# natir/br

Hardware: AMD Instinct MI355X
Metric: corrected Gbases/sec at k=19, 10 kb ONT-error reads (higher is better)
Workload: dtype u64 k-mers / 1-bit set

## Files before the change

br_amd/csrc/brx_correct.hip:

```cpp
#include "brx_correct.hpp"
#include <chrono>

#include <stdlib.h>
#include <string.h>
#include <algorithm>
#include <type_traits>
#include <thread>
#include <vector>

using namespace brx;

namespace brx {
uint64_t scan_tmp_bytes(uint32_t n);
int exclusive_scan_lens(const uint32_t *d_lens, uint32_t n, uint64_t *d_tmp, uint64_t *d_out_offsets,
                        unsigned long long *d_total, hipStream_t s);
int upload_batch(const uint8_t *bases, const uint64_t *offsets, uint32_t n_reads, uint8_t **d_bases, uint64_t *bases_cap,
                 uint64_t **d_off, uint64_t *off_cap, uint64_t *total, hipStream_t stream);
}

namespace {

enum { ST_INIT = 0, ST_SCAN, ST_ERRLEN, ST_ALTS, ST_SCEN, ST_MORE, ST_WALK, ST_T1, ST_TSCORE, ST_TMORE, ST_GFOLLOW, ST_GVALID };
enum { MODE_ONE = 0, MODE_GRAPH = 1, MODE_INSSUB = 2, MODE_TWO = 3 };

// ... 340 lines not shown
            }
            const uint64_t s0 = slot_of(o0, r, p.slack), s1 = slot_of(o1, (uint64_t)r + 1, p.slack);
            out = p.out + s0;
            cap = (uint32_t)(s1 - s0);
            st = ST_INIT;
            i = 0;
            olen = 0;
            kmer = 0;
            prev = false;
            steps = 0;
            skip_until = 0;
            if (VERIFY) {
                i = tr.i;
                olen = tr.i;
                uint64_t km = 0;
                for (int j = 0; j < k; j++)
                    km = (km << 2) | nuc2bit(in[p.flip ? (n - 1u - (tr.i + 1u - (uint32_t)k + (uint32_t)j)) : (tr.i + 1u - (uint32_t)k + (uint32_t)j)]);
                kmer = km;
                ch_t = in[p.flip ? (n - 1u - tr.i) : tr.i];
                elen = tr.elen;
                fc = tr.fc;
                if (HAS_TWO)
                    mode = MODE_TWO;
                else if (M == BRX_GRAPH)
                    mode = MODE_GRAPH;
                else if (M == BRX_GAP_SIZE) {
                    mode = elen < (uint32_t)k ? MODE_GRAPH : (elen == (uint32_t)k ? MODE_ONE : MODE_INSSUB);
                    gap = elen > (uint32_t)k ? elen - (uint32_t)k : 0u;
                } else
                    mode = MODE_ONE;
                st = ST_ALTS;
            }
            return;
        }
    };
    auto ld = [&](uint32_t j) -> uint8_t { return in[p.flip ? (n - 1u - j) : j]; };
    int done = 0;
    bool flag_read = false;
    auto end_read = [&](int how) {
        if (VERIFY && how != 1) {
            flag_read = true;
            done = 1;
        } else {
            done = how;
        }
    };
    auto finish = [&]() { end_read(1); };
    auto overflow = [&]() { end_read(16 + CTL_OVERFLOW); };
    auto nonterminating = [&]() { end_read(16 + CTL_NONTERM); };
    auto path_overflow = [&]() { end_read(16 + CTL_PATHOVF); };
    auto lane_kmer = [&](uint64_t carry, uint64_t code) -> uint64_t {
        uint64_t val = code;
#pragma unroll
        for (int d = 1; d < G && d < 32; d <<= 1) {
            const uint64_t other = __shfl_up(val, d, G);
            if (gl >= d)
                val |= other << (2 * d);
        }
        const int nb = gl + 1;
        return (nb >= k) ? (val & mask) : (((carry << (2 * nb)) | val) & mask);
    };

    constexpr int WB = G < 32 ? G : 32;
    auto group_window = [&](uint64_t code) -> uint64_t {
        uint64_t val = code;
#pragma unroll
        for (int d = 1; d < WB; d <<= 1) {
            const uint64_t other = __shfl_up(val, d, G);
            if (gl >= d)
                val |= other << (2 * d);
        }
        return __shfl(val, gshift + WB - 1);
    };
    auto ext = [&](uint64_t km, uint64_t W, uint32_t b0, uint32_t nb) -> uint64_t {
        const uint64_t bits = (W >> (2u * ((uint32_t)WB - b0 - nb))) & ((1ull << (2u * nb)) - 1ull);
        return ((km << (2u * nb)) | bits) & mask;
    };
    uint64_t win = 0;

    fetch();

    while (__any(have)) {
        if (G == 64) {
            while (have && st == ST_SCAN && !slow && n - i >= 65u && olen + 66u <= cap) {
                const uint8_t c8 = ld(i + (uint32_t)lane);
                const uint64_t km = lane_kmer64_dpp(kmer, (uint32_t)nuc2bit(c8), lane, mask);
                bool s1 = false;
                if (HAS_ERRLEN && i + (uint32_t)lane < skip_until) {
                } else if (p.idx.lines) {
                    s1 = index_get(p.idx, p.bits, km, k);
                } else {
                    s1 = probe(p.bits, km, k);
                }
                const uint64_t bs = __ballot(s1);
                const uint64_t trig = ~bs & ((bs << 1) | (prev ? 1ull : 0ull));
                if (trig)
                    break;
                out[olen + (uint32_t)lane] = c8;
                olen += 64u;
                i += 64u;
                kmer = ((uint64_t)(uint32_t)__builtin_amdgcn_readlane((int)(uint32_t)(km >> 32), 63) << 32) |
                       (uint32_t)__builtin_amdgcn_readlane((int)(uint32_t)km, 63);
                prev = (bs >> 63) & 1ull;
                n_rounds += 1u;
                n_probes += 64u;
                steps++;
            }
            while (HAS_ERRLEN && have && st == ST_ERRLEN && !slow && n - i > ej + 1u + 64u) {
                const uint8_t c8 = ld(i + ej + 1u + (uint32_t)lane);
                const uint64_t km = lane_kmer64_dpp(ek, (uint32_t)nuc2bit(c8), lane, mask);
                const bool s1 = p.idx.lines ? index_get(p.idx, p.bits, km, k) : probe(p.bits, km, k);
                if (__ballot(s1))
                    break;
                ek = ((uint64_t)(uint32_t)__builtin_amdgcn_readlane((int)(uint32_t)(km >> 32), 63) << 32) |
                     (uint32_t)__builtin_amdgcn_readlane((int)(uint32_t)km, 63);
                ej += 64u;
                n_rounds += 1u;
                n_probes += 64u;
                steps++;
            }
        }
        if (HAS_WALK) {
            constexpr uint64_t LEADERS = G == 64 ? 1ull : (G == 32 ? 0x0000000100000001ull : (G == 16 ? 0x0001000100010001ull : (G == 8 ? 0x0101010101010101ull : 0x1111111111111111ull)));
            for (uint32_t it = 0;; it++) {
                const bool wfast = have && st == ST_WALK && !slow && (brent || mode == MODE_INSSUB);
                const uint32_t nw = (uint32_t)__builtin_popcountll(__ballot(wfast) & LEADERS);
                const uint32_t no = (uint32_t)__builtin_popcountll(__ballot(have && !wfast) & LEADERS);
                if (nw == 0u || nw < no || (no != 0u && it >= 8u))
                    break;
                bool s1 = false, u1 = false;
                if (wfast && gl < 4) {
                    const uint64_t q = add_nuc(wk, (uint64_t)gl, mask);
                    if (p.idx.lines) {
                        const int pr = index_probe(p.idx, q, k);
                        s1 = pr == 1;
                        u1 = pr == 2;
                    } else {
                        s1 = probe(p.bits, q, k);
                    }
                }
                if (__ballot(u1))
                    break;
                const uint32_t am = (uint32_t)((__ballot(s1) >> gshift) & 0xfull);
                bool simple = wfast && __popc(am) == 1;
                uint64_t nk = 0;
                if (simple) {
                    nk = add_nuc(wk, (uint64_t)(__ffs(am) - 1), mask);
                    simple = !(brent && nk == tort) && !(!brent && npath >= p.maxpath) &&
                             !(mode == MODE_GRAPH ? nk == fc : gap <= 1u) && steps < (1u << 24) + 64u * n;
                }
                if (simple) {
                    if (brent && ++blam == bpow) {
                        tort = nk;
                        bpow *= 2u;
                        blam = 0;
                    }
                    if (gl == 0 && npath < p.maxpath)
                        __hip_atomic_store(path + npath, (unsigned long long)nk, __ATOMIC_RELAXED, __HIP_MEMORY_SCOPE_AGENT);
                    if (npath < 0xfffffff0u)
                        npath++;
                    wk = nk;
                    if (mode != MODE_GRAPH)
                        gap--;
                    steps++;
                }
                n_rounds += nw;
// ... 773 lines not shown
            if (cc)
                atomicAdd(p.ctrl + CTL_TRIGGERS, (unsigned long long)cc);
            if (d)
                atomicAdd(p.ctrl + CTL_FIXES, (unsigned long long)d);
        }
        ev = 0;
        since_flush = 0;
    };

    auto fetch = [&]() {
        for (;;) {
            unsigned long long w = 0;
            if (gl == 0)
                w = atomicAdd(p.ctrl + CTL_WORK, 1ull);
            w = __shfl(w, gshift);
            if (w >= (LIST ? *p.only_n : (unsigned long long)p.n_reads)) {
                have = false;
                return;
            }
            have = true;
            r = LIST ? p.only[w] : (uint32_t)w;
            const uint64_t o0 = p.offsets[r], o1 = p.offsets[r + 1];
            if (p.in_staged) {
                in = p.in + slot_of(o0, r, p.slack);
                n = p.in_lens[r];
                if (n == 0xffffffffu) {
                    if (gl == 0)
                        p.out_lens[r] = 0xffffffffu;
                    continue;
                }
            } else {
                in = p.in + o0;
                n = (uint32_t)(o1 - o0);
            }
            const uint64_t s0 = slot_of(o0, r, p.slack), s1 = slot_of(o1, (uint64_t)r + 1, p.slack);
            out = p.out + s0;
            cap = (uint32_t)(s1 - s0);
            st = ST_INIT;
            i = 0;
            olen = 0;
            kmer = 0;
            prev = false;
            steps = 0;
            return;
        }
    };
    auto ld = [&](uint32_t j) -> uint8_t { return in[p.flip ? (n - 1u - j) : j]; };
    int done = 0;
    auto finish = [&]() { done = 1; };
    auto give_up = [&](int which) { done = 16 + which; };
    auto lane_kmer = [&](uint64_t carry, uint32_t code, uint32_t &scan_out) -> uint64_t {
        if (G == 4) {
            const uint32_t v = row_scan4(code) & ((1u << nb2) - 1u);
            scan_out = v;
            return ((carry << nb2) | v) & mask;
        } else if (G == 8) {
            const uint32_t v = row_scan8(code) & ((1u << nb2) - 1u);
            scan_out = v;
            return ((carry << nb2) | v) & mask;
        } else if (G == 16) {
            const uint32_t v = row_scan16(code);
            scan_out = v;
            return ((carry << nb2) | v) & mask;
        } else {
            scan_out = 0;
            return lane_kmer64_dpp(carry, code, lane, mask);
        }
    };
    auto ext = [&](uint64_t km, uint32_t b0, uint32_t nb) -> uint64_t {
        const uint64_t bits = (uint64_t)((win >> (2u * ((uint32_t)WB - b0 - nb))) & (decltype(win))((1ull << (2u * nb)) - 1ull));
        return ((km << (2u * nb)) | bits) & mask;
    };

    fetch();

    while (__any(have)) {
        lane = lane0;
        asm volatile("" : "+v"(lane));
        gl = lane & (G - 1);
        gshift = lane & ~(G - 1);
        bcast_addr = (uint32_t)(lane | (G - 1)) * 4u;
        nb2 = 2u * ((uint32_t)gl + 1u);
        if (G == 64) {
            while (have && st == ST_SCAN && !slow && n - i >= 65u && olen + 66u <= cap) {
                const uint8_t c8 = ld(i + (uint32_t)lane);
                uint32_t sc;
                const uint64_t km = lane_kmer(kmer, (uint32_t)nuc2bit(c8), sc);
                const bool s1 = p.idx.lines ? index_get(p.idx, p.bits, km, k) : probe(p.bits, km, k);
                const uint64_t bs = __ballot(s1);
                const uint64_t trig = ~bs & ((bs << 1) | (prev ? 1ull : 0ull));
                if (trig)
                    break;
                out[olen + (uint32_t)lane] = c8;
                olen += 64u;
                i += 64u;
                kmer = ((uint64_t)(uint32_t)__builtin_amdgcn_readlane((int)(uint32_t)(km >> 32), 63) << 32) |
                       (uint32_t)__builtin_amdgcn_readlane((int)(uint32_t)km, 63);
                prev = (bs >> 63) & 1ull;
                ev += ((lane == 0) ? 1u : 0u) + (1u << 8);
                steps++;
                if (++since_flush == 255u)
                    flush();
            }
        }
        bool do_probe = false;
        uint64_t pk = 0;
        uint8_t ch = 0;
        uint32_t sc_s = 0, scan = 0, gwin = 0;
        bool sc_active = false;

        if (have) {
            ev += (gl == 0) ? 1u : 0u;
            if (st == ST_SCAN) {
                const uint32_t pos = i + (uint32_t)gl;
                const bool valid = pos < n;
                if (G < 64)
                    ch = pf_ch;
                else
                    ch = valid ? ld(pos) : (uint8_t)0;
                pk = lane_kmer(kmer, (uint32_t)nuc2bit(ch), scan);
                do_probe = valid;
                if (G <= 16)
                    gwin = (uint32_t)__builtin_amdgcn_ds_bpermute((int)bcast_addr, (int)scan);
            } else if (st == ST_INIT) {
                if (n < (uint32_t)k) {
                    for (uint32_t j = gl; j < n; j += G)
                        out[j] = ld(j);
                    olen = n;
                } else {
                    uint64_t km = 0;
                    for (int j = 0; j < k; j++)
                        km = (km << 2) | nuc2bit(ld((uint32_t)j));
                    kmer = km;
                    for (uint32_t j = gl; j < (uint32_t)k; j += G)
                        out[j] = ld(j);
                    olen = (uint32_t)k;
                    i = (uint32_t)k;
                    do_probe = (gl == 0);
                    pk = kmer;
                }
            } else if (st == ST_ALTS) {
                do_probe = gl < 4 && (uint64_t)gl != (kmer & 3ull);
                pk = (kmer & ~3ull) | (uint64_t)gl;
                if (G == 4) {
                    const uint32_t w4 = i + 4u * (uint32_t)gl;
                    uint32_t raw = 0;
                    if (w4 + 4u <= n) {
                        const uint8_t *q = p.flip ? in + (n - 4u - w4) : in + w4;
                        __builtin_memcpy(&raw, q, 4);
                        if (p.flip)
                            raw = __builtin_bswap32(raw);
                    } else {
                        for (uint32_t t = 0; t < 4u && w4 + t < n; t++)
                            raw |= (uint32_t)ld(w4 + t) << (8u * t);
                    }
                    uint32_t v = ((((raw >> 1) & 0x03030303u) * 0x40100401u) >> 24);
                    v |= dpp_row_shr<1>(v) << 8;
                    v |= dpp_row_shr<2>(v) << 16;
                    if (gl != 3)
                        v &= (1u << (8u * ((uint32_t)gl + 1u))) - 1u;
                    win = (uint32_t)__builtin_amdgcn_ds_bpermute((int)bcast_addr, (int)v);
                }
                const uint32_t wp = i + (uint32_t)gl;
                const uint32_t cd = (G != 4 && gl < WB && wp < n) ? (uint32_t)nuc2bit(ld(wp)) : 0u;
                if (G == 4) {
                } else if (G == 8) {
                    const uint32_t v = row_scan8(cd) & ((1u << nb2) - 1u);
                    win = (uint32_t)__builtin_amdgcn_ds_bpermute((int)bcast_addr, (int)v);
                } else if (G == 16) {
                    win = (uint32_t)__builtin_amdgcn_ds_bpermute((int)bcast_addr, (int)row_scan16(cd));
                } else {
                    const uint32_t v = row_scan16(cd);
                    const uint32_t w0 = (uint32_t)__builtin_amdgcn_readlane((int)v, 15), w1 = (uint32_t)__builtin_amdgcn_readlane((int)v, 31);
                    win = ((uint64_t)w0 << 32) | w1;
                }
            } else if (st == ST_SCEN && (G == 8 || G == 16)) {
                uint32_t off, j;
                if (sub == 0u) {
                    sc_s = (uint32_t)gl >> 1;
                    j = (uint32_t)gl & 1u;
                    sc_active = gl < 6 && !((failmask >> sc_s) & 1u) && j < c;
                } else {
                    sc_s = (uint32_t)__ffs(7u & ~failmask & ~passmask) - 1u;
                    j = sub + (uint32_t)gl;
                    sc_active = j < c;
                }
                off = 2u - sc_s;
                if (sc_active) {
                    if (c + 3u <= (uint32_t)WB) {
                        pk = ext(corr, off, j + 1u);
                    } else {
                        pk = corr;
                        for (uint32_t q = 0; q <= j; q++)
                            pk = add_nuc(pk, nuc2bit(ld(i + off + q)), mask);
                    }
                    do_probe = true;
                }
            } else if (st == ST_SCEN) {
                const uint32_t width = scen_width(sub, c, G, 0u, failmask);
                const uint32_t e = (uint32_t)gl;
                const uint32_t alive = ~failmask & 7u;
                const uint32_t ord = (e >= width ? 1u : 0u) + (e >= 2u * width ? 1u : 0u);
                sc_active = e < 3u * width && ord < (uint32_t)__popc(alive);
                const uint32_t a1 = alive & (alive - 1u);
                sc_s = !sc_active ? 0u : (ord == 0u ? (uint32_t)__ffs(alive) - 1u : (ord == 1u ? (uint32_t)__ffs(a1) - 1u : 2u));
                const uint32_t j = sub + (sc_active ? e - ord * width : 0u);
                const uint32_t off = 2u - sc_s;
                if (sc_active) {
                    if (c + 3u <= (uint32_t)WB) {
                        pk = ext(corr, off, j + 1u);
                    } else {
                        pk = corr;
                        for (uint32_t q = 0; q <= j; q++)
                            pk = add_nuc(pk, nuc2bit(ld(i + off + q)), mask);
                    }
                    do_probe = true;
                }
            } else {
// ... 202 lines not shown
                if (__popc(keep) == 1)
                    apply_s = __ffs(keep) - 1;
                else
                    fail = true;
            }
            if (have && steps > (1u << 24) + 64u * n) {
                fail = false;
                apply_s = -1;
                give_up(CTL_NONTERM);
            }
            if (fail) {
                if (olen + 2u > cap) {
                    give_up(CTL_OVERFLOW);
                } else {
                    if (gl == 0)
                        out[olen] = ld(i);
                    olen += 1;
                    i += 1;
                    prev = false;
                    if (i >= n)
                        finish();
                    else
                        st = ST_SCAN;
                }
            } else if (apply_s >= 0) {
                if (olen + 2u > cap) {
                    give_up(CTL_OVERFLOW);
                } else {
                    if (gl == 0)
                        out[olen] = bit2nuc(corr & 3ull);
                    olen += 1;
                    kmer = corr;
                    prev = true;
                    const uint32_t off = 2u - (uint32_t)apply_s;
                    i += off;
                    ev += (gl == 0) ? (1u << 24) : 0u;
                    if (c > 0u && c + 3u <= (uint32_t)WB && olen + c + 1u <= cap) {
                        for (uint32_t q = (uint32_t)gl; q < c; q += (uint32_t)G)
                            out[olen + q] = ld(i + q);
                        kmer = ext(kmer, off, c);
                        olen += c;
                        i += c;
                    }
                    if (i >= n)
                        finish();
                    else
                        st = ST_SCAN;
                }
            }
        }
        if (G < 64 && have && !done && !retry && st == ST_SCAN) {
            const uint32_t pos = i + (uint32_t)gl;
            pf_ch = pos < n ? ld(pos) : (uint8_t)0;
        }
        if (done) {
            if (gl == 0) {
                p.out_lens[r] = done == 1 ? olen : 0xffffffffu;
                if (done != 1)
                    atomicAdd(p.ctrl + (done - 16), 1ull);
            }
            done = 0;
            fetch();
        }
        if (++since_flush == 255u)
            flush();
    }
    flush();
}

#ifndef BRX_REV_WAVES
#define BRX_REV_WAVES 7
#endif
template <int KT, int M>
__global__ __launch_bounds__(256, BRX_REV_WAVES) void rev_scan_kernel(const PassParams pp, uint32_t *__restrict__ handback, uint32_t *__restrict__ redo_flag,
                                                                          TrigRec *__restrict__ notes, uint32_t trig_cap)
{
    const IdxView idx = pp.idx;
    const uint32_t *const bits = pp.bits;
    unsigned long long *const ctrl = pp.ctrl;
    const uint32_t n_reads = pp.n_reads, slack = pp.slack;
    const uint64_t *const offsets = pp.offsets;
    const uint8_t *const in_base = pp.in;
    const uint32_t *const in_lens = pp.in_lens;
    const bool in_staged = pp.in_staged != 0, flip = pp.flip != 0;
    uint8_t *const out_base = pp.out;
    uint32_t *const out_lens = pp.out_lens;
    constexpr bool HAS_ERRLEN = (M == BRX_GRAPH || M == BRX_GAP_SIZE);
    const int lane = threadIdx.x & 63;
    const int k = KT ? KT : pp.k;
    const uint64_t mask = kmask(k);
    uint32_t n_rounds = 0, n_probes = 0, n_trig = 0;

    auto ask = [&](uint64_t km) __attribute__((always_inline)) -> bool { return idx.lines ? index_get(idx, bits, km, k) : probe(bits, km, k); };
    auto last_of = [&](uint64_t km, uint32_t l) __attribute__((always_inline)) -> uint64_t {
        return ((uint64_t)(uint32_t)__builtin_amdgcn_readlane((int)(uint32_t)(km >> 32), (int)l) << 32) |
               (uint32_t)__builtin_amdgcn_readlane((int)(uint32_t)km, (int)l);
    };

    for (;;) {
        unsigned long long w = 0;
        if (lane == 0)
            w = atomicAdd(ctrl + CTL_WORK, 1ull);
        const uint32_t r = (uint32_t)__builtin_amdgcn_readfirstlane((int)(uint32_t)w);
        if (__builtin_amdgcn_readfirstlane((int)(uint32_t)(w >> 32)) != 0 || r >= n_reads)
            break;
        const uint64_t o0 = offsets[r], o1 = offsets[r + 1];
        const uint8_t *in;
        uint32_t n;
        if (in_staged) {
            in = in_base + slot_of(o0, r, slack);
            n = in_lens[r];
            if (n == 0xffffffffu) {
                if (lane == 0)
                    out_lens[r] = 0xffffffffu;
                continue;
            }
        } else {
            in = in_base + o0;
            n = (uint32_t)(o1 - o0);
        }
        const uint64_t s0 = slot_of(o0, r, slack), s1 = slot_of(o1, (uint64_t)r + 1, slack);
        uint8_t *out = out_base + s0;
        const uint32_t cap = (uint32_t)(s1 - s0);
        auto ld = [&](uint32_t j) __attribute__((always_inline)) -> uint8_t { return in[flip ? (n - 1u - j) : j]; };

        if (n < (uint32_t)k) {
            for (uint32_t j = (uint32_t)lane; j < n; j += 64u)
                out[j] = ld(j);
            if (lane == 0)
                out_lens[r] = n;
            continue;
        }
        bool hb = n + 1u > cap;
        uint64_t kmer = 0;
        uint32_t i = (uint32_t)k, skip_until = 0, trig_read = 0;
        bool prev = false;
        if (!hb) {
            for (int j = 0; j < k; j++)
                kmer = (kmer << 2) | nuc2bit(ld((uint32_t)j));
            if (lane < k)
                out[lane] = ld((uint32_t)lane);
            prev = ask(kmer);
            n_rounds++;
            n_probes++;
        }
        while (!hb && i < n) {
            const uint32_t pos = i + (uint32_t)lane;
            const bool valid = pos < n;
            const uint8_t c8 = valid ? ld(pos) : (uint8_t)0;
            const uint64_t km = lane_kmer64_dpp(kmer, (uint32_t)nuc2bit(c8), lane, mask);
            const bool asks = valid && !(HAS_ERRLEN && pos < skip_until);
            const bool a1 = asks && ask(km);
            n_rounds++;
            n_probes += (uint32_t)__builtin_popcountll(__ballot(asks));
            const uint32_t left = n - i;
            const uint32_t cnt = left < 64u ? left : 64u;
            const uint64_t vmask = cnt >= 64u ? ~0ull : ((1ull << cnt) - 1ull);
            const uint64_t bs = __ballot(a1);
            const uint64_t trig = ~bs & ((bs << 1) | (prev ? 1ull : 0ull)) & vmask;
            if (!trig) {
                if (valid)
                    out[pos] = c8;
                kmer = last_of(km, cnt - 1u);
                prev = (bs >> (cnt - 1u)) & 1ull;
                i += cnt;
                continue;
            }
            const uint32_t t = (uint32_t)__builtin_ctzll(trig);
            if ((uint32_t)lane < t)
                out[pos] = c8;
            i += t;
            kmer = last_of(km, t);
            trig_read++;
            uint32_t elen = 0;
            uint64_t fc = 0;
            bool hit_end = false;
            if (HAS_ERRLEN) {
                uint64_t ek = kmer;
                uint32_t ej = 0;
                const uint32_t rem = n - i;
                for (;;) {
                    const uint32_t j = ej + 1u + (uint32_t)lane;
                    const bool v2 = j < rem;
                    const uint8_t c2 = v2 ? ld(i + j) : (uint8_t)0;
                    const uint64_t km2 = lane_kmer64_dpp(ek, (uint32_t)nuc2bit(c2), lane, mask);
                    const bool a2 = v2 && ask(km2);
                    n_rounds++;
                    n_probes += (uint32_t)__builtin_popcountll(__ballot(v2));
                    const uint64_t sm = __ballot(a2);
                    if (sm) {
                        const uint32_t t2 = (uint32_t)__builtin_ctzll(sm);
                        elen = ej + 1u + t2;
                        fc = last_of(km2, t2);
                        break;
                    }
                    if (rem <= ej + 1u + 64u) {
                        const uint32_t nv = rem - (ej + 1u);
                        elen = rem;
                        fc = nv ? last_of(km2, nv - 1u) : ek;
                        hit_end = true;
                        break;
                    }
                    ek = last_of(km2, 63u);
                    ej += 64u;
                }
            }
            const bool none_already = HAS_ERRLEN && hit_end && (M == BRX_GRAPH || elen < (uint32_t)k);
            if (!none_already) {
                const bool asks3 = lane < 4 && (uint64_t)lane != (kmer & 3ull);
                const bool a3 = asks3 && ask(add_nuc(kmer >> 2, (uint64_t)(lane & 3), mask));
                n_rounds++;
                n_probes += 3u;
                if (__builtin_popcountll(__ballot(a3)) == 1) {
                    unsigned long long at = 0;
                    if (lane == 0)
                        at = atomicAdd(ctrl + CTL_REV_TRIGS, 1ull);
                    const uint32_t at_lo = (uint32_t)__builtin_amdgcn_readfirstlane((int)(uint32_t)at);
                    if (__builtin_amdgcn_readfirstlane((int)(uint32_t)(at >> 32)) != 0 || at_lo >= trig_cap) {
                        hb = true;
                        break;
                    }
                    if (lane == 0) {
                        notes[at_lo] = TrigRec{r, i, elen, 0u, fc};
                        atomicAdd(ctrl + CTL_REV_TRIGS_SUM, 1ull);
                    }
                }
            }
            if (lane == 0)
                out[i] = ld(i);
// ... 220 lines not shown
                correct_kernel<8, M, 2><<<blocks, 256, lds, s>>>(p);
            return BRX_OK;
        }
        if (p.only) {
            correct_kernel<64, M, 1><<<blocks, 256, lds, s>>>(p);
            return BRX_OK;
        }
    }
    if (lds > 64 * 1024) {
        const void *fn = G == 16 ? (const void *)correct_kernel<16, M>
                       : G == 32 ? (const void *)correct_kernel<32, M> : (const void *)correct_kernel<64, M>;
        BRX_HIP(hipFuncSetAttribute(fn, hipFuncAttributeMaxDynamicSharedMemorySize, (int)lds));
    }
    if (G <= 8 && M == BRX_ONE)
        correct_kernel<8, BRX_ONE><<<blocks, 256, lds, s>>>(p);
    else if (G == 4 && (M == BRX_GRAPH || M == BRX_GAP_SIZE))
        correct_kernel<4, (M == BRX_GRAPH || M == BRX_GAP_SIZE) ? M : BRX_GRAPH><<<blocks, 256, lds, s>>>(p);
    else if (G == 8 && (M == BRX_GRAPH || M == BRX_GAP_SIZE))
        correct_kernel<8, (M == BRX_GRAPH || M == BRX_GAP_SIZE) ? M : BRX_GRAPH><<<blocks, 256, lds, s>>>(p);
    else if (G <= 16)
        correct_kernel<16, M><<<blocks, 256, lds, s>>>(p);
    else if (G == 32)
        correct_kernel<32, M><<<blocks, 256, lds, s>>>(p);
    else
        correct_kernel<64, M><<<blocks, 256, lds, s>>>(p);
    return BRX_OK;
}

int greedy_group(int G, int k, int max_search, uint32_t *dim, uint32_t *per_group)
{
    *dim = (uint32_t)(k + max_search + 2);
    *per_group = greedy_lds_bytes(*dim);
    for (; G <= 64; G *= 2)
        if ((uint64_t)(256 / G) * *per_group <= 160u * 1024u)
            return G;
    return 0;
}

int launch_pass(PassParams p, const brx_method_t &md, int G, hipStream_t s)
{
    static const char *names[5] = {"correct_pass", "correct_pass_two", "correct_pass_graph", "correct_pass_greedy",
                                   "correct_pass_gap_size"};
    const int method = md.method;
    size_t lds = 0;
    p.max_search = md.max_search;
    {
        const char *e = getenv("BRX_TUNE");
        p.flags = e ? (uint32_t)atoi(e) : 0u;
    }
    p.g_dim = 0;
    p.g_lds_bytes = 0;
    if (method == BRX_GREEDY) {
        G = greedy_group(G, p.k, md.max_search, &p.g_dim, &p.g_lds_bytes);
        if (!G) {
            set_error("greedy: k=%d with max_search=%d needs a %u x %u alignment table that does not fit LDS", p.k,
                      (int)md.max_search, p.g_dim, p.g_dim);
            return BRX_ERR_UNSUPPORTED;
        }
        lds = (size_t)(256 / G) * p.g_lds_bytes;
    }
    uint32_t blocks = pass_blocks(p.n_reads, G, method == BRX_ONE);
    if (p.only || p.trig) {
        const uint64_t sized_groups = sized_path_lists(p.n_reads);
        const uint32_t per_block = p.trig ? 256u / (uint32_t)verify_group() : 4u;
        blocks = (uint32_t)(sized_groups / per_block);
        blocks = blocks < 1u ? 1u : (blocks > MAX_BLOCKS ? MAX_BLOCKS : blocks);
    }
    KernelTimer t(p.trig ? "rev_verify" : (p.only ? "rev_redo" : names[method]), s);
    switch (method) {
    case BRX_ONE: BRX_TRY(launch_method<BRX_ONE>(p, G, blocks, lds, s)); break;
    case BRX_TWO: BRX_TRY(launch_method<BRX_TWO>(p, G, blocks, lds, s)); break;
    case BRX_GRAPH: BRX_TRY(launch_method<BRX_GRAPH>(p, G, blocks, lds, s)); break;
    case BRX_GREEDY: BRX_TRY(launch_method<BRX_GREEDY>(p, G, blocks, lds, s)); break;
    case BRX_GAP_SIZE: BRX_TRY(launch_method<BRX_GAP_SIZE>(p, G, blocks, lds, s)); break;
    default: break;
    }
    BRX_HIP(hipGetLastError());
    return BRX_OK;
}

bool rev_lean_on()
{
    const char *e = getenv("BRX_REV_LEAN");
    return !(e && *e == '0');
}

template <int M>
void launch_rev_scan(const PassParams &p, uint32_t *list, uint32_t *flag, TrigRec *trig, uint32_t trig_cap, uint32_t blocks, hipStream_t s)
{
    if (p.k == 19)
        rev_scan_kernel<19, M><<<blocks, 256, 0, s>>>(p, list, flag, trig, trig_cap);
    else if (p.k == 21)
        rev_scan_kernel<21, M><<<blocks, 256, 0, s>>>(p, list, flag, trig, trig_cap);
    else
        rev_scan_kernel<0, M><<<blocks, 256, 0, s>>>(p, list, flag, trig, trig_cap);
}

int launch_rev_lean(brx_chain *ch, PassParams p, const brx_method_t &md, hipStream_t s)
{
    static const char *names[5] = {"correct_pass", "correct_pass_two", "correct_pass_graph", "correct_pass_greedy",
                                   "correct_pass_gap_size"};
    const uint64_t trig_cap64 = 4ull * p.n_reads + 4096ull;
    const uint32_t trig_cap = trig_cap64 > 0x7fffffffull ? 0x7fffffffu : (uint32_t)trig_cap64;
    BRX_TRY(ensure((void **)&ch->d_rev_list, &ch->rev_list_bytes, (uint64_t)p.n_reads * 4ull));
    BRX_TRY(ensure((void **)&ch->d_rev_flag, &ch->rev_flag_bytes, (uint64_t)p.n_reads * 4ull));
    BRX_TRY(ensure(&ch->d_rev_trig, &ch->rev_trig_bytes, (uint64_t)trig_cap * sizeof(TrigRec)));
    BRX_HIP(hipMemsetAsync(p.ctrl + CTL_REV_HANDBACK, 0, 8, s));
    BRX_HIP(hipMemsetAsync(p.ctrl + CTL_REV_TRIGS, 0, 8, s));
    BRX_HIP(hipMemsetAsync(ch->d_rev_flag, 0, (uint64_t)p.n_reads * 4ull, s));
    TrigRec *trig = (TrigRec *)ch->d_rev_trig;
    {
        const uint32_t blocks = pass_blocks(p.n_reads, 64);
        KernelTimer t(names[md.method], s);
        switch (md.method) {
        case BRX_ONE: launch_rev_scan<BRX_ONE>(p, ch->d_rev_list, ch->d_rev_flag, trig, trig_cap, blocks, s); break;
        case BRX_GRAPH: launch_rev_scan<BRX_GRAPH>(p, ch->d_rev_list, ch->d_rev_flag, trig, trig_cap, blocks, s); break;
        case BRX_GAP_SIZE: launch_rev_scan<BRX_GAP_SIZE>(p, ch->d_rev_list, ch->d_rev_flag, trig, trig_cap, blocks, s); break;
        default: set_error("launch_rev_lean: method %u", md.method); return BRX_ERR_ARG;
        }
        BRX_HIP(hipGetLastError());
    }
    PassParams v = p;
    v.trig = trig;
    v.trig_cap = trig_cap;
    v.only_n = p.ctrl + CTL_REV_TRIGS;
    v.redo_list = ch->d_rev_list;
    v.redo_flag = ch->d_rev_flag;
    BRX_HIP(hipMemsetAsync(p.ctrl + CTL_WORK, 0, 8, s));
    BRX_TRY(launch_pass(v, md, 16, s));
    p.only = ch->d_rev_list;
    p.only_n = p.ctrl + CTL_REV_HANDBACK;
    BRX_HIP(hipMemsetAsync(p.ctrl + CTL_WORK, 0, 8, s));
    return launch_pass(p, md, 16, s);
}

}

extern "C" {

int brx_chain_new(const brx_set_t *set, const brx_method_t *methods, uint32_t n_methods, bool two_side,
                  brx_chain_t **out)
{
    return brx_chain_new_pass(set, methods, n_methods, two_side ? BRX_PASS_NONE : BRX_PASS_REVERSE, out);
}

int brx_chain_second_pass(const brx_chain_t *ch)
{
    if (!ch) {
        set_error("null argument");
        return BRX_ERR_ARG;
    }
    return ch->second_pass;
}

int brx_chain_new_pass(const brx_set_t *set, const brx_method_t *methods, uint32_t n_methods, int second_pass,
                       brx_chain_t **out)
{
    if (!set || !out || (!methods && n_methods)) {
        set_error("null argument");
        return BRX_ERR_ARG;
    }
    if (second_pass != BRX_PASS_NONE && second_pass != BRX_PASS_REVERSE && second_pass != BRX_PASS_REVCOMP) {
        set_error("unknown second-pass mode %d (0 none, 1 reverse, 2 revcomp)", second_pass);
        return BRX_ERR_ARG;
    }
    for (uint32_t m = 0; m < n_methods; m++)
// ... 182 lines not shown
                BRX_TRY(ensure_bits(ch->set, s, "correction"));
                break;
            }
    BRX_TRY(index_ensure(ch->set, s));
    IdxView idx{nullptr, 0, 0, 0};
    if (ch->set->idx_valid && (index_wanted(k) || no_bits(ch->set)))
        idx = IdxView{ch->set->d_lines, 32u - ch->set->idx_log_lines, ch->set->idx_m, (uint32_t)k - ch->set->idx_m + 1u,
                      ch->set->idx_linebits ? (const uint32_t *)(ch->set->d_lines + (8ull << ch->set->idx_log_lines)) : nullptr};
    if (const char *e = getenv("BRX_LINE_BITS"))
        if (*e == '0')
            idx.line_bits = nullptr;

    const int n_dirs = ch->two_side ? 1 : 2;
    const bool revcomp = ch->second_pass == BRX_PASS_REVCOMP;
    const int n_methods = (int)ch->methods.size();
    uint64_t stats[8] = {0, 0, 0, 0, 0, 0, 0, 0};
    std::vector<SideRead> side;
    const int G = group_width(false, idx.lines != nullptr, n_reads);
    bool needs_path = false;
    for (int m = 0; m < n_methods; m++)
        needs_path |= (ch->methods[m].method == BRX_GRAPH || ch->methods[m].method == BRX_GAP_SIZE ||
                       ch->methods[m].method == BRX_GREEDY);
    uint32_t maxpath = ch->maxpath_seen;

    for (uint32_t slack = ch->slack_seen, attempt = 0;; attempt++) {
        if (attempt > 12) {
            set_error("correction output / graph walks do not fit the workspace after 12 enlargements; giving up");
            return BRX_ERR_OVERFLOW;
        }
        if (needs_path) {
            const uint64_t n_groups = sized_path_lists(n_reads);
            BRX_TRY(ensure((void **)&ch->d_path, &ch->path_bytes, n_groups * maxpath * 8ull));
        }
        const uint64_t stage_need = total_bases + (total_bases >> 2) * slack + 64ull * ((uint64_t)n_reads + 1) + 64;
        if (stage_need > ch->stage_bytes || !ch->d_stage[0]) {
            for (int q = 0; q < 2; q++) {
                if (ch->d_stage[q])
                    (void)hipFree(ch->d_stage[q]);
                ch->d_stage[q] = nullptr;
            }
            ch->stage_bytes = 0;
            BRX_HIP(hipMalloc((void **)&ch->d_stage[0], stage_need));
            BRX_HIP(hipMalloc((void **)&ch->d_stage[1], stage_need));
            ch->stage_bytes = stage_need;
        }

        const uint8_t *cur = d_bases;
        const uint32_t *cur_lens = nullptr;
        int cur_staged = 0, cur_rev = 0, pp = 0;
        bool any_overflow = false;
        BRX_HIP(hipMemsetAsync(ch->d_ctrl, 0, CTL_N * 8, s));
        for (int scan = 0; scan < n_dirs && !any_overflow; scan++) {
            const int dir = revcomp ? 0 : scan;
            if (revcomp && scan == 1 && cur_staged) {
                revcomp_stage(cur, cur_lens, d_offsets, n_reads, slack, ch->d_stage[pp], ch->d_lens[pp], s);
                cur = ch->d_stage[pp];
                cur_lens = ch->d_lens[pp];
                pp ^= 1;
            }
            for (int m = 0; m < n_methods; m++) {
                PassParams p;
                p.bits = no_bits(ch->set) ? nullptr : ch->set->d_bits;
                const int mth = ch->methods[m].method;
                const char *e_fwd = getenv("BRX_INDEX_FWD");
                const unsigned idx_fwd = e_fwd ? (unsigned)atoi(e_fwd) : 29u;
                const bool use_idx = no_bits(ch->set) || ((idx_fwd >> mth) & 1u) || (dir == 1 && mth != BRX_GREEDY);
                p.idx = use_idx ? idx : IdxView{nullptr, 0, 0, 0};
                p.k = k;
                p.c = ch->methods[m].confirm;
                p.n_reads = n_reads;
                p.offsets = d_offsets;
                p.in = cur;
                p.in_lens = cur_lens;
                p.in_staged = cur_staged;
                p.flip = (cur_rev != dir);
                p.out = ch->d_stage[pp];
                p.out_lens = ch->d_lens[pp];
                p.slack = slack;
                p.ctrl = (unsigned long long *)ch->d_ctrl;
                p.path_k = ch->d_path;
                p.maxpath = maxpath;
                BRX_HIP(hipMemsetAsync(ch->d_ctrl + CTL_WORK, 0, 8, s));
                p.flags = 0;
                p.max_search = 0;
                p.g_dim = 0;
                p.g_lds_bytes = 0;
                const unsigned lane_rev_default = 0u;
                const char *e_rev = getenv("BRX_LANE_REV");
                const unsigned lane_rev = e_rev && *e_rev ? (unsigned)atoi(e_rev) : lane_rev_default;
                const bool lane_dir = dir == 0 ? !p.flip
                                               : ((mth == BRX_GRAPH && (lane_rev & 1u)) || (mth == BRX_GAP_SIZE && (lane_rev & 2u)));
                if ((mth == BRX_ONE || mth == BRX_GRAPH || mth == BRX_GAP_SIZE) && lane_dir) {
                    const LanePassInfo info{cur_staged ? ch->stage_bytes : total_bases, mth};
                    const int lst = lane_pass(ch, p, info, s);
                    if (lst != BRX_OK && lst != BRX_ERR_UNSUPPORTED)
                        return lst;
                    if (lst == BRX_OK) {
                        cur = ch->d_stage[pp];
                        cur_lens = ch->d_lens[pp];
                        cur_staged = 1;
                        cur_rev = dir;
                        pp ^= 1;
                        continue;
                    }
                }
                int gw = dir ? group_width(true, false, n_reads) : G;
                if (gw < 16 && mth != BRX_ONE) {
                    gw = (mth == BRX_GRAPH || mth == BRX_GAP_SIZE) ? walk_group() : 16;
                }
                const char *e_lo = getenv("BRX_REV_LEAN_ONE");
                const bool lean_one = mth == BRX_ONE && e_lo && *e_lo == '1';
                const bool lean = dir == 1 && (mth == BRX_GRAPH || mth == BRX_GAP_SIZE || lean_one) && gw == 64 && rev_lean_on();
                if (lean)
                    BRX_TRY(launch_rev_lean(ch, p, ch->methods[m], s));
                else
                    BRX_TRY(launch_pass(p, ch->methods[m], gw, s));
                cur = ch->d_stage[pp];
                cur_lens = ch->d_lens[pp];
                cur_staged = 1;
                cur_rev = dir;
                pp ^= 1;
            }
        }
        if (n_methods == 0) {
            set_error("empty method list");
            return BRX_ERR_ARG;
        }
        static const bool tr_attempts = [] { const char *e = getenv("BRX_TRACE"); return e && *e == '1'; }();
        if (tr_attempts)
            fprintf(stderr, "[brx correct] attempt %u launched: slack %u maxpath %u n_reads %u\n", attempt, slack, maxpath, n_reads);
        BRX_HIP(hipMemcpyAsync(ch->h_ctrl, ch->d_ctrl, CTL_N * 8, hipMemcpyDeviceToHost, s));
        BRX_HIP(hipStreamSynchronize(s));
        if (tr_attempts)
            fprintf(stderr, "[brx correct] attempt %u done: slot overflows %llu, walk list overflows %llu, nonterminating %llu, "
                            "lean reverse passes: %llu open triggers verified, %llu reads redone\n", attempt,
                    (unsigned long long)ch->h_ctrl[CTL_OVERFLOW], (unsigned long long)ch->h_ctrl[CTL_PATHOVF],
                    (unsigned long long)ch->h_ctrl[CTL_NONTERM], (unsigned long long)ch->h_ctrl[CTL_REV_TRIGS_SUM],
                    (unsigned long long)ch->h_ctrl[CTL_REV_HANDBACK_SUM]);
        stats[4] = attempt;
        if (ch->h_ctrl[CTL_NONTERM] != 0) {
            set_error("%llu read(s): the scan does not terminate (e.g. greedy moving the read cursor backwards for ever; "
                      "the reference spins on such input)", (unsigned long long)ch->h_ctrl[CTL_NONTERM]);
            return BRX_ERR_UNSUPPORTED;
        }
        if (ch->h_ctrl[CTL_OVERFLOW] != 0 || ch->h_ctrl[CTL_PATHOVF] != 0) {
            stats[5] += ch->h_ctrl[CTL_OVERFLOW];
            stats[6] += ch->h_ctrl[CTL_PATHOVF];
            bool patched = false;
            if (ch->h_ctrl[CTL_OVERFLOW] + ch->h_ctrl[CTL_PATHOVF] <= redo_max_reads()) {
                side.clear();
                const int rst = redo_poisoned_reads(ch, d_bases, d_offsets, n_reads, const_cast<uint8_t *>(cur),
                                                    const_cast<uint32_t *>(cur_lens), cur_rev, slack,
                                                    ch->h_ctrl[CTL_OVERFLOW] ? slack * 4u : slack,
                                                    ch->h_ctrl[CTL_PATHOVF] ? maxpath * 8u : maxpath, side, s);
                if (rst == BRX_OK) {
                    patched = true;
                    if (ch->sub)
                        for (int q = 0; q < 4; q++)
                            stats[q] += ch->sub->last_stats[q];
                }
                else if (rst != BRX_ERR_UNSUPPORTED)
                    return rst;
            }
            if (!patched) {
                side.clear();
                if (ch->h_ctrl[CTL_OVERFLOW] != 0)
// ... 277 lines not shown
```

br_amd/csrc/brx_correct.hpp:

```cpp
#pragma once
#include "brx_internal.hpp"
#include "brx_index.hpp"

namespace brx {

enum { CTL_WORK = 0, CTL_OVERFLOW = 1, CTL_ROUNDS = 2, CTL_PROBES = 3, CTL_TRIGGERS = 4, CTL_FIXES = 5, CTL_TOTAL = 6, CTL_PATHOVF = 7, CTL_NONTERM = 8,
       CTL_LANE_UNITS = 9, CTL_LANE_MISS = 10, CTL_LANE_WORK = 11, CTL_LANE_FAIL = 12,
       CTL_REV_HANDBACK = 13, CTL_REV_HANDBACK_SUM = 14,
       CTL_LANE_UNWRITTEN = 15,
       CTL_REV_TRIGS = 16, CTL_REV_TRIGS_SUM = 17,
       CTL_AP_VEC = 18, CTL_AP_BYTEWAY = 19, CTL_AP_PARTIAL = 20,
       CTL_N = 21 };

struct TrigRec {
    uint32_t r;
    uint32_t i;
    uint32_t elen;
    uint32_t pad;
    uint64_t fc;
};

struct PassParams {
    const uint32_t *bits;
    IdxView idx;
    int k;
    int c;
    uint32_t n_reads;
    const uint64_t *offsets;
    const uint8_t *in;
    const uint32_t *in_lens;
    int in_staged;
    int flip;
    uint8_t *out;
    uint32_t *out_lens;
    uint32_t slack;
    unsigned long long *ctrl;
    uint64_t *path_k;
    uint32_t maxpath;
    uint32_t flags;
    int max_search;
    uint32_t g_dim;
    uint32_t g_lds_bytes;
    const uint32_t *only = nullptr;
    const unsigned long long *only_n = nullptr;
    const TrigRec *trig = nullptr;
    uint32_t trig_cap = 0;
    uint32_t *redo_list = nullptr;
    uint32_t *redo_flag = nullptr;
};

__host__ __device__ __forceinline__ uint64_t slot_of(uint64_t o, uint64_t r, uint32_t slack)
{
    return o + (o >> 2) * (uint64_t)slack + 64ull * r;
}

__device__ __forceinline__ bool probe(const uint32_t *__restrict__ bits, uint64_t fwd, int k)
{
    const uint64_t h = khash(fwd, k);
    return (bits[h >> 5] >> (h & 31u)) & 1u;
}


#if defined(__HIPCC__)
template <int D>
__device__ __forceinline__ uint32_t dpp_row_shr(uint32_t v)
{
    return (uint32_t)__builtin_amdgcn_update_dpp(0, (int)v, 0x110 + D, 0xf, 0xf, true);
}

__device__ __forceinline__ uint32_t row_scan16(uint32_t code)
{
    uint32_t v = code;
    v |= dpp_row_shr<1>(v) << 2;
    v |= dpp_row_shr<2>(v) << 4;
    v |= dpp_row_shr<4>(v) << 8;
    v |= dpp_row_shr<8>(v) << 16;
    return v;
}
__device__ __forceinline__ uint64_t lane_kmer64_dpp(uint64_t carry, uint32_t code, int lane, uint64_t mask)
{
    const uint32_t v = row_scan16(code);
    const uint32_t clo = (uint32_t)carry, chi = (uint32_t)(carry >> 32);
    const uint32_t b1 = (uint32_t)__builtin_amdgcn_update_dpp((int)clo, (int)v, 0x142 , 0xe, 0xf, false);
    const uint32_t old2 = (lane < 16) ? chi : clo;
    const uint32_t b2 = (uint32_t)__builtin_amdgcn_update_dpp((int)old2, (int)b1, 0x142, 0xc, 0xf, false);
    const uint32_t jb = 2u * ((uint32_t)(lane & 15) + 1u);
    return (((((uint64_t)b2 << 32) | b1) << jb) | v) & mask;
}

#endif

struct LanePassInfo {
    uint64_t in_total_bound;
    int method;
};
int lane_pass(brx_chain *ch, const PassParams &p, const LanePassInfo &info, hipStream_t s);
void lane_ws_free(brx_chain *ch);
int launch_one_list(const PassParams &p, hipStream_t s);
int launch_walk_list(const PassParams &p, int method, hipStream_t s);

}
```

Before: 26.65.

## Batch reverse-pass scan rounds with minimizer prefilter and compacted probe queue

Adds a block path for the reverse-direction scan. It processes several 64-base rounds per call, computes minimizer line hashes with DPP, and filters k-mers through a line-occupancy bitmap. Only surviving k-mers are compacted into an LDS queue and probed in dense waves, which cuts divergent index probes per round. The cost is possible wasted work when a trigger appears early in the block, plus extra LDS use. The change also builds the initial k-mer with a wave-parallel DPP scan in place of a serial loop.

```diff
diff --git a/br_amd/csrc/brx_correct.hip b/br_amd/csrc/brx_correct.hip
--- a/br_amd/csrc/brx_correct.hip
+++ b/br_amd/csrc/brx_correct.hip
@@ -446,6 +446,22 @@
 
     while (__any(have)) {
         if (G == 64) {
+            while (!HAS_GREEDY && p.rev_batch && have && st == ST_SCAN && !slow && n - i >= 64u * REV_BLOCK + 1u && olen + 64u * REV_BLOCK + 2u <= cap) {
+                const uint8_t *const in_b = (const uint8_t *)uni64((uint64_t)in);
+                uint8_t *const out_b = (uint8_t *)uni64((uint64_t)(out + olen));
+                const uint32_t n_b = uni32(n), i_b = uni32(i);
+                const bool flip_b = p.flip != 0;
+                const uint32_t t = rev_block_rounds<HAS_ERRLEN>(p.idx, p.bits, k, mask, lane,
+                                                                [in_b, n_b, flip_b](uint32_t j) -> uint8_t { return in_b[flip_b ? (n_b - 1u - j) : j]; }, i_b,
+                                                                out_b, uni32(skip_until), kmer, prev);
+                olen += 64u * t;
+                i += 64u * t;
+                n_rounds += t;
+                n_probes += 64u * t;
+                steps += t;
+                if (t < (uint32_t)REV_BLOCK)
+                    break;
+            }
             while (have && st == ST_SCAN && !slow && n - i >= 65u && olen + 66u <= cap) {
                 const uint8_t c8 = ld(i + (uint32_t)lane);
                 const uint64_t km = lane_kmer64_dpp(kmer, (uint32_t)nuc2bit(c8), lane, mask);
@@ -1385,6 +1401,24 @@
         bcast_addr = (uint32_t)(lane | (G - 1)) * 4u;
         nb2 = 2u * ((uint32_t)gl + 1u);
         if (G == 64) {
+            while (p.rev_batch && have && st == ST_SCAN && !slow && n - i >= 64u * REV_BLOCK + 1u && olen + 64u * REV_BLOCK + 2u <= cap) {
+                if (since_flush + REV_BLOCK >= 255u)
+                    flush();
+                const uint8_t *const in_b = (const uint8_t *)uni64((uint64_t)in);
+                uint8_t *const out_b = (uint8_t *)uni64((uint64_t)(out + olen));
+                const uint32_t n_b = uni32(n), i_b = uni32(i);
+                const bool flip_b = p.flip != 0;
+                const uint32_t t = rev_block_rounds<false>(p.idx, p.bits, k, mask, lane,
+                                                           [in_b, n_b, flip_b](uint32_t j) -> uint8_t { return in_b[flip_b ? (n_b - 1u - j) : j]; }, i_b,
+                                                           out_b, 0u, kmer, prev);
+                olen += 64u * t;
+                i += 64u * t;
+                ev += ((lane == 0) ? t : 0u) + (t << 8);
+                steps += t;
+                since_flush += t;
+                if (t < (uint32_t)REV_BLOCK)
+                    break;
+            }
             while (have && st == ST_SCAN && !slow && n - i >= 65u && olen + 66u <= cap) {
                 const uint8_t c8 = ld(i + (uint32_t)lane);
                 uint32_t sc;
@@ -1431,12 +1465,21 @@
                         out[j] = ld(j);
                     olen = n;
                 } else {
-                    uint64_t km = 0;
-                    for (int j = 0; j < k; j++)
-                        km = (km << 2) | nuc2bit(ld((uint32_t)j));
-                    kmer = km;
-                    for (uint32_t j = gl; j < (uint32_t)k; j += G)
-                        out[j] = ld(j);
+                    if (G == 64) {
+                        const uint8_t cj = lane < k ? ld((uint32_t)lane) : (uint8_t)0;
+                        const uint64_t kv = lane_kmer64_dpp(0ull, (uint32_t)nuc2bit(cj), lane, mask);
+                        kmer = ((uint64_t)(uint32_t)__builtin_amdgcn_readlane((int)(uint32_t)(kv >> 32), k - 1) << 32) |
+                               (uint32_t)__builtin_amdgcn_readlane((int)(uint32_t)kv, k - 1);
+                        if (lane < k)
+                            out[lane] = cj;
+                    } else {
+                        uint64_t km = 0;
+                        for (int j = 0; j < k; j++)
+                            km = (km << 2) | nuc2bit(ld((uint32_t)j));
+                        kmer = km;
+                        for (uint32_t j = gl; j < (uint32_t)k; j += G)
+                            out[j] = ld(j);
+                    }
                     olen = (uint32_t)k;
                     i = (uint32_t)k;
                     do_probe = (gl == 0);
@@ -1805,7 +1848,7 @@
     const uint64_t *const offsets = pp.offsets;
     const uint8_t *const in_base = pp.in;
     const uint32_t *const in_lens = pp.in_lens;
-    const bool in_staged = pp.in_staged != 0, flip = pp.flip != 0;
+    const bool in_staged = pp.in_staged != 0, flip = pp.flip != 0, rev_batch = pp.rev_batch != 0;
     uint8_t *const out_base = pp.out;
     uint32_t *const out_lens = pp.out_lens;
     constexpr bool HAS_ERRLEN = (M == BRX_GRAPH || M == BRX_GAP_SIZE);
@@ -1868,6 +1911,20 @@
             n_probes++;
         }
         while (!hb && i < n) {
+            if (rev_batch && n - i >= 64u * REV_BLOCK + 1u) {
+                const uint32_t t = rev_block_rounds<HAS_ERRLEN>(idx, bits, k, mask, lane,
+                                                                [in, n, flip](uint32_t j) -> uint8_t { return in[flip ? (n - 1u - j) : j]; }, i,
+                                                                out + i, skip_until, kmer, prev);
+                for (uint32_t q = 0; q < t; q++) {
+                    const uint32_t p0 = i + 64u * q;
+                    const uint32_t skipped = (HAS_ERRLEN && skip_until > p0) ? (skip_until - p0 < 64u ? skip_until - p0 : 64u) : 0u;
+                    n_probes += 64u - skipped;
+                }
+                n_rounds += t;
+                i += 64u * t;
+                if (t == (uint32_t)REV_BLOCK)
+                    continue;
+            }
             const uint32_t pos = i + (uint32_t)lane;
             const bool valid = pos < n;
             const uint8_t c8 = valid ? ld(pos) : (uint8_t)0;
@@ -2254,6 +2311,12 @@
 bool rev_lean_on()
 {
     const char *e = getenv("BRX_REV_LEAN");
+    return !(e && *e == '0');
+}
+
+bool rev_batch_on()
+{
+    const char *e = getenv("BRX_REV_BATCH");
     return !(e && *e == '0');
 }
 
@@ -2602,6 +2665,7 @@
                 p.maxpath = maxpath;
                 BRX_HIP(hipMemsetAsync(ch->d_ctrl + CTL_WORK, 0, 8, s));
                 p.flags = 0;
+                p.rev_batch = (dir == 1 && !revcomp && rev_batch_on() && rev_block_applies(p.idx)) ? 1 : 0;
                 p.max_search = 0;
                 p.g_dim = 0;
                 p.g_lds_bytes = 0;
diff --git a/br_amd/csrc/brx_correct.hpp b/br_amd/csrc/brx_correct.hpp
--- a/br_amd/csrc/brx_correct.hpp
+++ b/br_amd/csrc/brx_correct.hpp
@@ -47,6 +47,7 @@
     uint32_t trig_cap = 0;
     uint32_t *redo_list = nullptr;
     uint32_t *redo_flag = nullptr;
+    int rev_batch = 0;
 };
 
 __host__ __device__ __forceinline__ uint64_t slot_of(uint64_t o, uint64_t r, uint32_t slack)
@@ -87,7 +88,143 @@
     const uint32_t jb = 2u * ((uint32_t)(lane & 15) + 1u);
     return (((((uint64_t)b2 << 32) | b1) << jb) | v) & mask;
 }
-
+#endif
+
+#ifndef BRX_REV_BLOCK
+#define BRX_REV_BLOCK 4
+#endif
+constexpr int REV_BLOCK = BRX_REV_BLOCK;
+constexpr uint32_t REV_MAX_W = 8;
+constexpr uint32_t REV_QUEUE = 128;
+static_assert(REV_BLOCK >= 1 && REV_BLOCK <= 16, "BRX_REV_BLOCK: 1 .. 16 rounds");
+
+inline bool rev_block_applies(const IdxView &v)
+{
+    return v.lines != nullptr && v.line_bits != nullptr && v.line_shift >= 6u && v.w >= 1u && v.w <= REV_MAX_W;
+}
+
+#if defined(__HIPCC__)
+__device__ __forceinline__ uint32_t mmer_hash(uint32_t f, uint32_t m)
+{
+    uint32_t x = __brev(f ^ 0xAAAAAAAAu);
+    x = ((x >> 1) & 0x55555555u) | ((x & 0x55555555u) << 1);
+    const uint32_t r = x >> (32u - 2u * m);
+    return (f < r ? f : r) * 0x9E3779B1u;
+}
+
+__device__ __forceinline__ uint32_t uni32(uint32_t v) { return (uint32_t)__builtin_amdgcn_readfirstlane((int)v); }
+__device__ __forceinline__ uint64_t uni64(uint64_t v) { return ((uint64_t)uni32((uint32_t)(v >> 32)) << 32) | uni32((uint32_t)v); }
+
+template <bool HAS_SKIP, typename LD>
+__device__ __forceinline__ uint32_t rev_block_rounds(const IdxView &idx, const uint32_t *__restrict__ bits, int k, uint64_t mask, int lane0, LD ld,
+                                                     uint32_t i, uint8_t *__restrict__ outp, uint32_t skip_until, uint64_t &kmer, bool &prev)
+{
+    __shared__ uint4 rev_q[4][REV_QUEUE];
+    __shared__ unsigned long long rev_ans[4][2 * REV_BLOCK];
+    const uint32_t wv = uni32(threadIdx.x >> 6);
+    uint4 *const q = rev_q[wv];
+    unsigned long long *const ans = rev_ans[wv];
+    unsigned long long *const carry = ans + REV_BLOCK;
+    const uint32_t m = idx.m, w = idx.w;
+    const uint32_t mm = m >= 16u ? 0xffffffffu : (1u << (2u * m)) - 1u;
+
+    if (lane0 < REV_BLOCK)
+        ans[lane0] = 0ull;
+
+    uint32_t count = 0;
+    bool any_solid = false;
+    uint64_t cur_carry = uni64(kmer);
+    uint8_t c_next = ld(i + (uint32_t)lane0);
+#pragma unroll 1
+    for (uint32_t r = 0; r < (uint32_t)REV_BLOCK; r++) {
+        {
+            int ln = lane0;
+            asm volatile("" : "+v"(ln));
+            const uint8_t c8 = c_next;
+            if (r + 1u < (uint32_t)REV_BLOCK)
+                c_next = ld(i + 64u * (r + 1u) + (uint32_t)ln);
+            const uint64_t carry_in = cur_carry;
+            const uint64_t km = lane_kmer64_dpp(cur_carry, (uint32_t)nuc2bit(c8), ln, mask);
+            outp[64u * r + (uint32_t)ln] = c8;
+            if (ln == 63)
+                carry[r] = km;
+            cur_carry = ((uint64_t)(uint32_t)__builtin_amdgcn_readlane((int)(uint32_t)(km >> 32), 63) << 32) |
+                        (uint32_t)__builtin_amdgcn_readlane((int)(uint32_t)km, 63);
+            const uint32_t h = mmer_hash((uint32_t)km & mm, m);
+            uint32_t best = h, cur = h;
+#pragma unroll
+            for (uint32_t s = 1; s < REV_MAX_W; s++)
+                if (s < w) {
+                    const uint32_t front = mmer_hash((uint32_t)(carry_in >> (2u * (s - 1u))) & mm, m);
+                    cur = (uint32_t)__builtin_amdgcn_update_dpp((int)front, (int)cur, 0x138 , 0xf, 0xf, false);
+                    best = cur < best ? cur : best;
+                }
+            const uint32_t home = index_line_of(best, idx.line_shift);
+            bool occ = (idx.line_bits[home >> 5] >> (home & 31u)) & 1u;
+            if (HAS_SKIP && i + 64u * r + (uint32_t)ln < skip_until)
+                occ = false;
+            const uint64_t em = __ballot(occ);
+            if (occ) {
+                const uint32_t rank = __builtin_amdgcn_mbcnt_hi((uint32_t)(em >> 32), __builtin_amdgcn_mbcnt_lo((uint32_t)em, 0u));
+                q[count + rank] = make_uint4((uint32_t)km, (uint32_t)(km >> 32), home, (r << 6) | (uint32_t)ln);
+            }
+            count += (uint32_t)__builtin_popcountll(em);
+            __builtin_amdgcn_wave_barrier();
+        }
+        while (count > REV_QUEUE - 64u || (r + 1u == (uint32_t)REV_BLOCK && count)) {
+            const uint32_t cnt = count < 64u ? count : 64u;
+            bool sol = false;
+            int ln = lane0;
+            asm volatile("" : "+v"(ln));
+            if ((uint32_t)ln < cnt) {
+                const uint4 e = q[count - cnt + (uint32_t)ln];
+                const uint64_t fwd = ((uint64_t)e.y << 32) | e.x;
+                const uint64_t rc = revcomp(fwd, k);
+                const uint64_t key = (((popc64(fwd) & 1) ? rc : fwd) >> 1) + 1ull;
+                int a = index_probe_at(idx, key, e.z, 0u);
+                if (a == 2) {
+                    if (bits) {
+                        const uint64_t hh = key - 1ull;
+                        a = (bits[hh >> 5] >> (hh & 31u)) & 1u;
+                    } else {
+                        const uint32_t last = 0xffffffffu >> idx.line_shift;
+                        for (uint32_t hop = 1; a == 2 && hop <= last; hop++)
+                            a = index_probe_at(idx, key, e.z, hop);
+                    }
+                }
+                sol = a == 1;
+            }
+            if (__ballot(sol)) {
+                any_solid = true;
+                if (sol) {
+                    const uint32_t tag = q[count - cnt + (uint32_t)ln].w;
+                    atomicOr(ans + (tag >> 6), 1ull << (tag & 63u));
+                }
+            }
+            count -= cnt;
+            __builtin_amdgcn_wave_barrier();
+        }
+    }
+
+    uint32_t t = 0;
+    if (!any_solid) {
+        t = prev ? 0u : (uint32_t)REV_BLOCK;
+    } else {
+        bool pv = prev;
+        for (; t < (uint32_t)REV_BLOCK; t++) {
+            const uint64_t bs = uni64(ans[t]);
+            if (~bs & ((bs << 1) | (pv ? 1ull : 0ull)))
+                break;
+            pv = (bs >> 63) & 1ull;
+        }
+        if (t)
+            prev = pv;
+    }
+    if (t)
+        kmer = uni64(carry[t - 1u]);
+    __builtin_amdgcn_wave_barrier();
+    return t;
+}
 #endif
 
 struct LanePassInfo {
```

Result: no change. 27.25, median of 6 (+2.3%).
